# IRVLUTD/Proto-CLIP

Measured on AMD Instinct MI355X. Metric: query images/sec, ImageNet 16-shot ViT-B/16 (few-shot top-1 parity: tests/), higher is better.
Workload: dtype f16; 1 GPU; C3 ImageNet 16-shot ViT-B/16 conv-3x: prototype reduce + encode_image + adapter + dual-bank classify; batch_per_gpu=1024, global_batch=1024, classes=1000, shots=16, embed_dim=512, parallelism=dp1 (support rows and queries sharded; all-gather of class sums)

## Files before the change

### proto-clip_amd/csrc/pclip_attention.hip

```cpp
#include "pclip_attention_tile.h"
#include <stdlib.h>
#include <type_traits>

namespace {
constexpr int ATT_MAX_L = 288;

template <int NW, int VAR, bool QF = false>
__global__ __launch_bounds__(NW * 64, NW / 2) void attention_kernel(const half_t* __restrict__ qp, int ldq, long q_batch,
                                                           const half_t* __restrict__ kvp, int ldkv, int k_off, int v_off,
                                                           half_t* __restrict__ out, int L, int Lq, int H, int causal, int NT,
                                                           int LV) {
    extern __shared__ __attribute__((aligned(16))) char smem[];
    const int LP = NT * 32;
    half_t* Ks = reinterpret_cast<half_t*>(smem);
    half_t* Vs = Ks + LP * ATT_DH;
    const int b = blockIdx.x / H, h = blockIdx.x % H;
    const int W = H * ATT_DH;
    const half_t* kbase = kvp + (size_t)b * L * ldkv + h * ATT_DH + k_off;
    const half_t* vbase = kvp + (size_t)b * L * ldkv + h * ATT_DH + v_off;
    const half_t* qbase = qp + (size_t)b * q_batch + h * ATT_DH;
    const int tid = threadIdx.x, lane = tid & 63, wave = tid >> 6;
    half8_t qf0[4];
    if (QF) {
        const int q0 = wave * 32 + (lane & 31), qc0 = q0 < Lq ? q0 : Lq - 1;
#pragma unroll
        for (int s_ = 0; s_ < 4; ++s_) qf0[s_] = ld_half8(qbase + (size_t)qc0 * ldq + s_ * 16 + (lane >> 5) * 8);
    }

    for (int r0 = wave * 8; r0 < LP; r0 += NW * 8) {
        const int r = r0 + (lane >> 3);
        const int c = (lane & 7) ^ pgemm::swz_key(r);
        const int rc = r < L ? r : L - 1;
        __builtin_amdgcn_global_load_lds((pgemm::gbl_ptr_t)(kbase + (size_t)rc * ldkv + c * 8),
                                         (pgemm::lds_ptr_t)(Ks + r0 * ATT_DH), 16, 0, 0);
    }
    for (int r0 = wave * 8; r0 < LP; r0 += NW * 8) {
        const int r = r0 + (lane >> 3);
        const int c = (lane & 7) ^ (((r >> 1) & 1) << 2);
        const int rc = r < L ? r : L - 1;
        __builtin_amdgcn_global_load_lds((pgemm::gbl_ptr_t)(vbase + (size_t)rc * ldkv + c * 8),
                                         (pgemm::lds_ptr_t)(Vs + r0 * ATT_DH), 16, 0, 0);
    }
#ifndef PCLIP_ATT_VBAR
#define PCLIP_ATT_VBAR 1
#endif
    constexpr bool VB = PCLIP_ATT_VBAR && QF;
    if (VB) {
        const int nv = (LP - wave * 8 + NW * 8 - 1) / (NW * 8);
        if (nv <= 1) pgemm::wait_vm<1>(); else if (nv == 2) pgemm::wait_vm<2>(); else if (nv == 3) pgemm::wait_vm<3>(); else pgemm::wait_vm<4>();
        pgemm::lds_barrier();
    } else
        __syncthreads();

    const int hi = lane >> 5, ql = lane & 31;
    int voff[2];
    attn_voff(lane, voff);
    const int NTq = (Lq + 31) >> 5;
    auto process = [&](int qb, const half8_t (&qf)[4]) {
        const int q = qb * 32 + ql;
        float16_t o[2];
        float lrun;
        attn_query_tile<false, VAR, VB>(Ks, Vs, qf, q, qb, L, causal, NT, hi, ql, voff, o, lrun);
        attn_store_tile(out + ((size_t)b * Lq + q) * W + h * ATT_DH, o, lrun, hi, q < Lq);
    };
    if (QF) {
        if (wave < NTq) process(wave, qf0);
        else if (VB) { pgemm::wait_vm<0>(); pgemm::lds_barrier(); }
        return;
    }
    for (int qb = wave; qb < NTq; qb += NW) {
        const int q = qb * 32 + ql;
        const int qc = q < Lq ? q : Lq - 1;
        half8_t qf[4];
#pragma unroll
        for (int s = 0; s < 4; ++s) qf[s] = ld_half8(qbase + (size_t)qc * ldq + s * 16 + hi * 8);
        process(qb, qf);
    }
}

template <int NW, int WPS, int VAR>
__global__ __launch_bounds__(NW * 64, WPS) void attention_pipe_kernel(const half_t* __restrict__ qp, int ldq, long q_batch,
                                                                      const half_t* __restrict__ kvp, int ldkv, int k_off, int v_off,
                                                                      half_t* __restrict__ out, int L, int H, int causal, int NT, int KR,
                                                                      int nitems) {
    extern __shared__ __attribute__((aligned(16))) char smem[];
    constexpr int NST = 4;
    constexpr int MAXP = 4;
    constexpr int RB = ATT_DH * 2;
    const int LP = NT * 32;
    const int BUF = (KR + LP) * RB;
    const int tid = threadIdx.x, lane = tid & 63, wave = __builtin_amdgcn_readfirstlane(tid >> 6);
    const int hi = lane >> 5, ql = lane & 31;
    const int W = H * ATT_DH, G = gridDim.x;
    const bool has_tile = wave < NT;
    const unsigned lds0 = (unsigned)(size_t)(pgemm::lds_ptr_t)smem;
    char* Qs = smem + 2 * BUF;
    int voff[2];
    attn_voff(lane, voff);
    int kvo[MAXP], vvo[MAXP], qvo[MAXP];
#pragma unroll
    for (int i = 0; i < MAXP; ++i) {
        const int r = wave * 8 + i * NW * 8 + (lane >> 3);
        const int rc = r < L ? r : L - 1;
        const int ck = ((lane & 7) ^ pgemm::swz_key(r)) << 3, cv = ((lane & 7) ^ (((r >> 1) & 1) << 2)) << 3;
        kvo[i] = (rc * ldkv + ck) * 2;
        vvo[i] = (rc * ldkv + cv) * 2;
        qvo[i] = (rc * ldq + ck) * 2;
    }
    const int q = wave * 32 + ql;
    auto stage = [&](int item, int buf) {
        const int b = item / H, h = item - b * H;
        const uint4_t rkv = attn_rsrc(kvp + (size_t)b * L * ldkv + h * ATT_DH);
        const uint4_t rq = attn_rsrc(qp + (size_t)b * q_batch + h * ATT_DH);
        const unsigned kb = lds0 + buf * BUF, vb = kb + KR * RB, qb = lds0 + 2 * BUF;
#pragma unroll
        for (int i = 0; i < MAXP; ++i) {
            const int r0 = wave * 8 + i * NW * 8;
            if (r0 < KR) attn_dma16(rkv, kvo[i], k_off * 2, kb + r0 * RB);
        }
#pragma unroll
        for (int i = 0; i < MAXP; ++i) {
            const int r0 = wave * 8 + i * NW * 8;
            if (r0 < LP) attn_dma16(rkv, vvo[i], v_off * 2, vb + r0 * RB);
        }
#pragma unroll
        for (int i = 0; i < MAXP; ++i) {
            const int r0 = wave * 8 + i * NW * 8;
            if (r0 < KR) attn_dma16(rq, qvo[i], 0, qb + r0 * RB);
        }
    };
    int item = blockIdx.x;
    if (item >= nitems) return;
    stage(item, 0);
    for (int it = 0; item < nitems; item += G, ++it) {
        const int cur = it & 1;
        if (has_tile && it > 0) pgemm::wait_vm<NST>(); else pgemm::wait_vm<0>();
        pgemm::lds_barrier();
        half8_t qf[4];
        if (has_tile) {
            const int qr = q < KR ? q : KR - 1;
#pragma unroll
            for (int s = 0; s < 4; ++s)
                qf[s] = *reinterpret_cast<const half8_t*>(Qs + qr * RB + (((s * 2 + hi) ^ pgemm::swz_key(qr)) << 4));
        }
        pgemm::lds_barrier();
#ifndef PCLIP_ATT_ABL
#define PCLIP_ATT_ABL 0
#endif
        const int next = item + G;
        if (next < nitems && !(PCLIP_ATT_ABL & 1)) stage(next, cur ^ 1);
        if (has_tile) {
            const half_t* Ks = reinterpret_cast<const half_t*>(smem + cur * BUF);
            const half_t* Vs = Ks + KR * ATT_DH;
            float16_t o[2];
            float lrun;
#ifndef PCLIP_ATT_STAGGER
#define PCLIP_ATT_STAGGER 0
#endif
#if PCLIP_ATT_STAGGER && defined(__HIP_DEVICE_COMPILE__)
            if (wave >= NW / 2) __builtin_amdgcn_s_sleep(PCLIP_ATT_STAGGER);
#endif
            if (PCLIP_ATT_ABL & 2) {
#pragma unroll
                for (int j = 0; j < 2; ++j)
#pragma unroll
                    for (int e = 0; e < 16; ++e) o[j][e] = (float)qf[e & 3][e & 7];
                lrun = 1.f;
            } else
                attn_query_tile<true, VAR>(Ks, Vs, qf, q, wave, L, causal, NT, hi, ql, voff, o, lrun);
            const int b = item / H, h = item - b * H;
            attn_store_tile(out + ((size_t)b * L + q) * W + h * ATT_DH, o, lrun, hi, q < L && !(PCLIP_ATT_ABL & 4));
        }
    }
}

}

static int att_mode_from_env() {
    const char* e = getenv("PCLIP_ATT_PIPE");
    return e && (e[0] == '0' || e[0] == '1') ? e[0] - '0' : -1;
}
static int g_att_mode = att_mode_from_env(), g_att_grid = 0;
extern "C" int pclip_attention_config(int mode, int max_grid) {
    PCLIP_REQUIRE(mode >= -1 && mode <= 1 && max_grid >= 0, "pclip_attention_config: bad mode=%d max_grid=%d", mode, max_grid);
    g_att_mode = mode;
    g_att_grid = max_grid;
    return PCLIP_OK;
}

extern "C" int pclip_attention_q_f16(const void* q, int ldq, long q_batch_stride, const void* kv, int ldkv, int k_off, int v_off,
                                     void* out, int B, int L, int Lq, int H, int dh, int causal, pclip_stream_t stream) {
    PCLIP_REQUIRE(q && kv && out, "pclip_attention_q_f16: null pointer");
    PCLIP_REQUIRE(dh == ATT_DH, "pclip_attention_q_f16: head dim %d unsupported (must be 64)", dh);
    PCLIP_REQUIRE(B >= 0 && H > 0 && L > 0 && L <= ATT_MAX_L && Lq > 0 && Lq <= L, "pclip_attention_q_f16: bad B=%d H=%d L=%d Lq=%d (L <= %d)",
                  B, H, L, Lq, ATT_MAX_L);
    PCLIP_REQUIRE(!causal || Lq == L, "pclip_attention_q_f16: the causal mask needs all queries (Lq == L)");
    PCLIP_REQUIRE(ldq % 8 == 0 && ldkv % 8 == 0 && k_off % 8 == 0 && v_off % 8 == 0 && q_batch_stride % 8 == 0,
                  "pclip_attention_q_f16: strides / offsets must be multiples of 8 halves");
    if (B == 0) return PCLIP_OK;
    const int NT = ceil_div(L, 32), LP = NT * 32;
    const int LV = 0;
    const long nitems = (long)B * H;
    const int cus = pclip_device_cus();
    const int KR = (L + 7) / 8 * 8;
    const size_t plds = (2 * (size_t)(KR + LP) + KR) * ATT_DH * 2;
    if (Lq == L && g_att_mode != 0 && NT <= 8 && plds <= 160 * 1024 && cus > 0 && g_att_mode == 1) {
        static DevOnce pipe_attr;
        if (!pipe_attr.done()) {
            if (hipFuncSetAttribute((const void*)attention_pipe_kernel<4, 2, PCLIP_ATT_VAR_SHORT>, hipFuncAttributeMaxDynamicSharedMemorySize, 160 * 1024) != hipSuccess ||
                hipFuncSetAttribute((const void*)attention_pipe_kernel<8, 2, PCLIP_ATT_VAR_LONG>, hipFuncAttributeMaxDynamicSharedMemorySize, 160 * 1024) != hipSuccess) {
                pclip_set_error("pclip_attention_f16: cannot raise the dynamic LDS limit");
                return PCLIP_E_LAUNCH;
            }
            pipe_attr.set();
        }
        int per_cu = NT <= 4 ? (int)((160 * 1024) / plds) : 1;
        per_cu = per_cu < 1 ? 1 : (per_cu > 2 ? 2 : per_cu);
        long grid = (long)cus * per_cu;
        if (g_att_grid > 0 && g_att_grid < grid) grid = g_att_grid;
        if (grid > nitems) grid = nitems;
        if (NT <= 4)
            attention_pipe_kernel<4, 2, PCLIP_ATT_VAR_SHORT><<<(int)grid, 256, plds, (hipStream_t)stream>>>((const half_t*)q, ldq, q_batch_stride, (const half_t*)kv, ldkv,
                                                                                      k_off, v_off, (half_t*)out, L, H, causal, NT, KR, (int)nitems);
        else
            attention_pipe_kernel<8, 2, PCLIP_ATT_VAR_LONG><<<(int)grid, 512, plds, (hipStream_t)stream>>>((const half_t*)q, ldq, q_batch_stride, (const half_t*)kv, ldkv,
                                                                                      k_off, v_off, (half_t*)out, L, H, causal, NT, KR, (int)nitems);
        return pclip_check_launch("attention (pipelined)");
    }
    const size_t lds = 2 * (size_t)LP * ATT_DH * 2;
    static DevOnce attr_set;
    if (!attr_set.done()) {
        const void* fns[] = {(const void*)attention_kernel<8, PCLIP_ATT_VAR_LONG>, (const void*)attention_kernel<4, PCLIP_ATT_VAR_LONG>,
                             (const void*)attention_kernel<4, PCLIP_ATT_VAR_SHORT>, (const void*)attention_kernel<8, PCLIP_ATT_VAR_LONG, true>,
                             (const void*)attention_kernel<4, PCLIP_ATT_VAR_SHORT, true>};
        for (const void* f : fns)
            if (hipFuncSetAttribute(f, hipFuncAttributeMaxDynamicSharedMemorySize, 80 * 1024) != hipSuccess) {
                pclip_set_error("pclip_attention_f16: cannot raise the dynamic LDS limit");
                return PCLIP_E_LAUNCH;
            }
        attr_set.set();
    }
#define PCLIP_ATT_LAUNCH(NW, VAR)                                                                                                         \
    attention_kernel<NW, VAR><<<B * H, NW * 64, lds, (hipStream_t)stream>>>((const half_t*)q, ldq, q_batch_stride, (const half_t*)kv, ldkv, k_off, \
                                                                             v_off, (half_t*)out, L, Lq, H, causal, NT, LV)
    static const bool qfirst = !(getenv("PCLIP_ATT_QFIRST") && getenv("PCLIP_ATT_QFIRST")[0] == '0');
    if (PCLIP_ATT_QF4 && qfirst && NT <= 4 && Lq == L && !causal)
        attention_kernel<4, PCLIP_ATT_VAR_SHORT, true><<<B * H, 4 * 64, lds, (hipStream_t)stream>>>((const half_t*)q, ldq, q_batch_stride, (const half_t*)kv, ldkv, k_off,
                                                                                                     v_off, (half_t*)out, L, Lq, H, causal, NT, LV);
    else if ((Lq + 31) / 32 > 4 && (Lq + 31) / 32 <= 8 && NT <= 8 && qfirst)
        attention_kernel<8, PCLIP_ATT_VAR_LONG, true><<<B * H, 8 * 64, lds, (hipStream_t)stream>>>((const half_t*)q, ldq, q_batch_stride, (const half_t*)kv, ldkv, k_off,
                                                                                                    v_off, (half_t*)out, L, Lq, H, causal, NT, LV);
    else if ((Lq + 31) / 32 > 4) PCLIP_ATT_LAUNCH(8, PCLIP_ATT_VAR_LONG);
    else if (NT > 4) PCLIP_ATT_LAUNCH(4, PCLIP_ATT_VAR_LONG);
    else PCLIP_ATT_LAUNCH(4, PCLIP_ATT_VAR_SHORT);
#undef PCLIP_ATT_LAUNCH
    return pclip_check_launch("attention");
}

extern "C" int pclip_attention_f16(const void* qkv, void* out, int B, int L, int H, int dh, int causal,
                                   pclip_stream_t stream) {
    PCLIP_REQUIRE(qkv && out, "pclip_attention_f16: null pointer");
    PCLIP_REQUIRE(H > 0 && L > 0, "pclip_attention_f16: bad H=%d L=%d", H, L);
    const int W = H * dh;
    return pclip_attention_q_f16(qkv, 3 * W, (long)L * 3 * W, qkv, 3 * W, W, 2 * W, out, B, L, L, H, dh, causal, stream);
}
```

### proto-clip_amd/csrc/pclip_attention_tile.h

```cpp
#pragma once
#include "pclip_encoder_common.h"
#include <type_traits>

namespace {
constexpr int ATT_DH = 64;
constexpr float kAttDefer = 2.f;
#ifndef PCLIP_ATT_VAR_LONG
#define PCLIP_ATT_VAR_LONG 15
#endif
#ifndef PCLIP_ATT_VAR_SHORT
#define PCLIP_ATT_VAR_SHORT 1
#endif

typedef __fp16 fp16x4_t __attribute__((__vector_size__(4 * sizeof(__fp16))));
__device__ __forceinline__ half4_t tr_read4(const char* lds_addr) {
    const fp16x4_t v = __builtin_amdgcn_ds_read_tr16_b64_v4f16((__attribute__((address_space(3))) fp16x4_t*)(lds_addr));
    return __builtin_bit_cast(half4_t, v);
}

__device__ __forceinline__ void attn_voff(int lane, int (&voff)[2]) {
    const int hi = lane >> 5;
    const int i16 = lane & 15, vrow = hi * 4 + (i16 >> 2), vd = ((lane >> 4) & 1) * 16 + 4 * (i16 & 3), vswz = ((vrow >> 1) & 1) << 2;
#pragma unroll
    for (int j = 0; j < 2; ++j) voff[j] = vrow * (ATT_DH * 2) + ((((j * 4 + (vd >> 3)) ^ vswz)) << 4) + (vd & 7) * 2;
}

__device__ __forceinline__ void half_wave_pair(float v, float& r0, float& r1) {
#if defined(__HIP_DEVICE_COMPILE__)
    const unsigned a = __builtin_bit_cast(unsigned, v);
    const auto r = __builtin_amdgcn_permlane32_swap(a, a, false, false);
    const unsigned x = r[0], y = r[1];
    r0 = __builtin_bit_cast(float, x);
    r1 = __builtin_bit_cast(float, y);
#else
    r0 = r1 = v;
#endif
}
__device__ __forceinline__ float half_wave_max(float v) { float a, b; half_wave_pair(v, a, b); return fmaxf(a, b); }
__device__ __forceinline__ float half_wave_sum(float v) { float a, b; half_wave_pair(v, a, b); return a + b; }

#ifndef PCLIP_ATT_QF4
#define PCLIP_ATT_QF4 1
#endif
#ifndef PCLIP_ATT_EDGE
#define PCLIP_ATT_EDGE 1
#endif
template <bool DEEP = false, int VAR = 0, bool VBAR = false>
__device__ __forceinline__ void attn_key_tiles(const half_t* Ks, const half_t* Vs, const half8_t (&qf)[4], int q, int qb, int L, int causal,
                                               int NT, int hi, int ql, const int (&voff)[2], float16_t (&o)[2],
                                               float& mrun_io, float& lrun_io) {
    constexpr float kScale = 0.125f * 1.4426950408889634f;
    float mrun = mrun_io, lrun = lrun_io;
    const int tend = causal ? (qb + 1 < NT ? qb + 1 : NT) : NT;
    auto k_frag = [&](int t, int sidx) {
        const int kr = t * 32 + ql;
        return *reinterpret_cast<const half8_t*>(Ks + kr * ATT_DH + (((sidx * 2 + hi) ^ pgemm::swz_key(kr)) << 3));
    };
    auto v_frag = [&](int t, int sidx, int j) {
        const char* vb = reinterpret_cast<const char*>(Vs) + (t * 32 + sidx * 16) * (ATT_DH * 2) + voff[j];
        const half4_t v0 = tr_read4(vb);
        const half4_t v1 = tr_read4(vb + 8 * (ATT_DH * 2));
        return half8_t{v0[0], v0[1], v0[2], v0[3], v1[0], v1[1], v1[2], v1[3]};
    };
    half8_t kpre[2][4];
    auto k_prefetch = [&](int t0) {
#pragma unroll
        for (int u = 0; u < 2; ++u) {
            const int tt = t0 + u < NT ? t0 + u : NT - 1;
#pragma unroll
            for (int sidx = 0; sidx < 4; ++sidx) kpre[u][sidx] = k_frag(tt, sidx);
        }
    };
    auto tiles = [&](auto NTILE_C, int t0) {
        constexpr int NTILE = decltype(NTILE_C)::value;
        float16_t st[NTILE];
#pragma unroll
        for (int u = 0; u < NTILE; ++u)
#pragma unroll
            for (int e = 0; e < 16; ++e) st[u][e] = 0.f;
#if defined(__HIP_DEVICE_COMPILE__)
        if (VAR & 8) __builtin_amdgcn_s_setprio(1);
#endif
#pragma unroll
        for (int sidx = 0; sidx < 4; ++sidx)
#pragma unroll
            for (int u = 0; u < NTILE; ++u) {
                const half8_t kf = DEEP ? kpre[u][sidx] : k_frag(t0 + u, sidx);
                st[u] = __builtin_amdgcn_mfma_f32_32x32x16_f16(kf, qf[sidx], st[u], 0, 0, 0);
            }
#if defined(__HIP_DEVICE_COMPILE__)
        if (VAR & 8) __builtin_amdgcn_s_setprio(0);
#endif
        half8_t vpre[NTILE][2][2];
        if (DEEP) {
#pragma unroll
            for (int u = 0; u < NTILE; ++u)
#pragma unroll
                for (int sidx = 0; sidx < 2; ++sidx)
#pragma unroll
                    for (int j = 0; j < 2; ++j) vpre[u][sidx][j] = v_frag(t0 + u, sidx, j);
            const int tn = t0 + NTILE;
            if (tn < tend) k_prefetch(tn);
#if defined(__HIP_DEVICE_COMPILE__)
            __builtin_amdgcn_sched_barrier(0);
#endif
        }
        float tmax = -__builtin_inff();
#pragma unroll
        for (int u = 0; u < NTILE; ++u) {
            const int t = t0 + u;
            if ((t * 32 + 32 > L) || (causal && t == qb)) {
                const int kend = causal ? (q + 1 < L ? q + 1 : L) : L;
                const int lim = kend - t * 32 - 4 * hi;
#pragma unroll
                for (int e = 0; e < 16; ++e)
                    if (!((e & 3) + 8 * (e >> 2) < lim)) st[u][e] = -__builtin_inff();
            }
        }
        {
            float m4[4] = {tmax, tmax, tmax, tmax};
#pragma unroll
            for (int u = 0; u < NTILE; ++u)
#pragma unroll
                for (int e = 0; e < 16; ++e) m4[e & 3] = fmaxf(m4[e & 3], st[u][e]);
            tmax = fmaxf(fmaxf(m4[0], m4[1]), fmaxf(m4[2], m4[3]));
        }
        tmax = half_wave_max(tmax) * kScale;
        const bool moved = (VAR & 1) ? tmax > mrun + kAttDefer : fmaxf(mrun, tmax) != mrun;
        const float mnew = ((VAR & 1) && !moved) ? mrun : fmaxf(mrun, tmax);
        const bool grow = __any(moved);
        float psum = 0.f;
        if (VAR & 6) {
            float2_t ps2 = {0.f, 0.f};
            const float2_t ks2 = {kScale, kScale}, nm2 = {-mnew, -mnew};
#pragma unroll
            for (int u = 0; u < NTILE; ++u)
#pragma unroll
                for (int e = 0; e < 16; e += 2) {
                    float2_t v = {st[u][e], st[u][e + 1]};
                    if (VAR & 4) {
                        v = v * ks2 + nm2;
                        v = float2_t{__builtin_amdgcn_exp2f(v[0]), __builtin_amdgcn_exp2f(v[1])};
                    } else
                        v = float2_t{__builtin_amdgcn_exp2f(fmaf(v[0], kScale, -mnew)), __builtin_amdgcn_exp2f(fmaf(v[1], kScale, -mnew))};
                    st[u][e] = v[0];
                    st[u][e + 1] = v[1];
                    if (VAR & 2) ps2 += v;
                    else { psum += v[0]; psum += v[1]; }
                }
            psum += ps2[0] + ps2[1];
        } else {
#pragma unroll
            for (int u = 0; u < NTILE; ++u)
#pragma unroll
                for (int e = 0; e < 16; ++e) { st[u][e] = __builtin_amdgcn_exp2f(fmaf(st[u][e], kScale, -mnew)); psum += st[u][e]; }
        }
        psum = half_wave_sum(psum);
        if (grow) {
            const float alpha = __builtin_amdgcn_exp2f(mrun - mnew);
            lrun *= alpha;
#pragma unroll
            for (int j = 0; j < 2; ++j)
#pragma unroll
                for (int e = 0; e < 16; ++e) o[j][e] *= alpha;
        }
        lrun += psum;
        mrun = mnew;
        if (VBAR && t0 == 0) { pgemm::wait_vm<0>(); pgemm::lds_barrier(); }
#pragma unroll
        for (int u = 0; u < NTILE; ++u)
#pragma unroll
            for (int sidx = 0; sidx < 2; ++sidx) {
                half8_t pf;
#pragma unroll
                for (int e = 0; e < 8; ++e) pf[e] = (half_t)st[u][sidx * 8 + e];
#if defined(__HIP_DEVICE_COMPILE__)
                if (VAR & 8) __builtin_amdgcn_s_setprio(1);
#endif
#pragma unroll
                for (int j = 0; j < 2; ++j) {
                    const half8_t vf = DEEP ? vpre[u][sidx][j] : v_frag(t0 + u, sidx, j);
                    o[j] = __builtin_amdgcn_mfma_f32_32x32x16_f16(vf, pf, o[j], 0, 0, 0);
                }
#if defined(__HIP_DEVICE_COMPILE__)
                if (VAR & 8) __builtin_amdgcn_s_setprio(0);
#endif
            }
    };
    auto tile_edge = [&](int t0) {
        const int ng = (L - t0 * 32 + 7) >> 3;
        float16_t st;
#pragma unroll
        for (int e = 0; e < 16; ++e) st[e] = 0.f;
#if defined(__HIP_DEVICE_COMPILE__)
        if (VAR & 8) __builtin_amdgcn_s_setprio(1);
#endif
#pragma unroll
        for (int sidx = 0; sidx < 4; ++sidx) st = __builtin_amdgcn_mfma_f32_32x32x16_f16(k_frag(t0, sidx), qf[sidx], st, 0, 0, 0);
#if defined(__HIP_DEVICE_COMPILE__)
        if (VAR & 8) __builtin_amdgcn_s_setprio(0);
#endif
        const int lim = L - t0 * 32 - 4 * hi;
        float m4[4] = {-__builtin_inff(), -__builtin_inff(), -__builtin_inff(), -__builtin_inff()};
#pragma unroll
        for (int g = 0; g < 3; ++g)
            if (g < ng) {
#pragma unroll
                for (int r = 0; r < 4; ++r) {
                    if (!(r + 8 * g < lim)) st[4 * g + r] = -__builtin_inff();
                    m4[r] = fmaxf(m4[r], st[4 * g + r]);
                }
            }
        float tmax = fmaxf(fmaxf(m4[0], m4[1]), fmaxf(m4[2], m4[3]));
        tmax = half_wave_max(tmax) * kScale;
        const bool moved = (VAR & 1) ? tmax > mrun + kAttDefer : fmaxf(mrun, tmax) != mrun;
        const float mnew = ((VAR & 1) && !moved) ? mrun : fmaxf(mrun, tmax);
        const bool grow = __any(moved);
        float psum = 0.f;
        float2_t ps2 = {0.f, 0.f};
        const float2_t ks2 = {kScale, kScale}, nm2 = {-mnew, -mnew};
#pragma unroll
        for (int g = 0; g < 4; ++g) {
            if (g < 3 && g < ng) {
#pragma unroll
                for (int e = 4 * g; e < 4 * g + 4; e += 2) {
                    float2_t v = {st[e], st[e + 1]};
                    if (VAR & 6) {
                        if (VAR & 4) {
                            v = v * ks2 + nm2;
                            v = float2_t{__builtin_amdgcn_exp2f(v[0]), __builtin_amdgcn_exp2f(v[1])};
                        } else
                            v = float2_t{__builtin_amdgcn_exp2f(fmaf(v[0], kScale, -mnew)), __builtin_amdgcn_exp2f(fmaf(v[1], kScale, -mnew))};
                        if (VAR & 2) ps2 += v;
                        else { psum += v[0]; psum += v[1]; }
                    } else {
                        v[0] = __builtin_amdgcn_exp2f(fmaf(v[0], kScale, -mnew)); psum += v[0];
                        v[1] = __builtin_amdgcn_exp2f(fmaf(v[1], kScale, -mnew)); psum += v[1];
                    }
                    st[e] = v[0];
                    st[e + 1] = v[1];
                }
            } else {
#pragma unroll
                for (int r = 0; r < 4; ++r) st[4 * g + r] = 0.f;
            }
        }
        if (VAR & 6) psum += ps2[0] + ps2[1];
        psum = half_wave_sum(psum);
        if (grow) {
            const float alpha = __builtin_amdgcn_exp2f(mrun - mnew);
            lrun *= alpha;
#pragma unroll
            for (int j = 0; j < 2; ++j)
#pragma unroll
                for (int e = 0; e < 16; ++e) o[j][e] *= alpha;
        }
        lrun += psum;
        mrun = mnew;
        if (VBAR && t0 == 0) { pgemm::wait_vm<0>(); pgemm::lds_barrier(); }
#pragma unroll
        for (int sidx = 0; sidx < 2; ++sidx)
            if (sidx == 0 || ng > 2) {
                half8_t pf;
#pragma unroll
                for (int e = 0; e < 8; ++e) pf[e] = (half_t)st[sidx * 8 + e];
#if defined(__HIP_DEVICE_COMPILE__)
                if (VAR & 8) __builtin_amdgcn_s_setprio(1);
#endif
#pragma unroll
                for (int j = 0; j < 2; ++j) o[j] = __builtin_amdgcn_mfma_f32_32x32x16_f16(v_frag(t0, sidx, j), pf, o[j], 0, 0, 0);
#if defined(__HIP_DEVICE_COMPILE__)
                if (VAR & 8) __builtin_amdgcn_s_setprio(0);
#endif
            }
    };
    int t = 0;
    if (DEEP) k_prefetch(0);
    for (; t + 1 < tend; t += 2) tiles(std::integral_constant<int, 2>{}, t);
    if (t < tend) {
        if (PCLIP_ATT_EDGE && VBAR && !DEEP && !causal && L - t * 32 <= 24) tile_edge(t);
        else tiles(std::integral_constant<int, 1>{}, t);
    }
    mrun_io = mrun;
    lrun_io = lrun;
}

template <bool DEEP = false, int VAR = 0, bool VBAR = false>
__device__ __forceinline__ void attn_query_tile(const half_t* Ks, const half_t* Vs, const half8_t (&qf)[4], int q, int qb, int L, int causal,
                                                int NT, int hi, int ql, const int (&voff)[2], float16_t (&o)[2], float& lrun_out) {
#pragma unroll
    for (int j = 0; j < 2; ++j)
#pragma unroll
        for (int e = 0; e < 16; ++e) o[j][e] = 0.f;
    float mrun = -__builtin_inff(), lrun = 0.f;
    attn_key_tiles<DEEP, VAR, VBAR>(Ks, Vs, qf, q, qb, L, causal, NT, hi, ql, voff, o, mrun, lrun);
    lrun_out = lrun;
}

__device__ __forceinline__ void attn_store_tile(half_t* orow, const float16_t (&o)[2], float lrun, int hi, bool valid) {
    const float inv = 1.f / lrun;
#pragma unroll
    for (int j = 0; j < 2; ++j)
#pragma unroll
        for (int k = 0; k < 2; ++k) {
            unsigned a[2], bq[2];
#pragma unroll
            for (int w = 0; w < 2; ++w) {
                const half2_t ha = {(half_t)(o[j][8 * k + 2 * w] * inv), (half_t)(o[j][8 * k + 2 * w + 1] * inv)};
                const half2_t hb = {(half_t)(o[j][8 * k + 4 + 2 * w] * inv), (half_t)(o[j][8 * k + 4 + 2 * w + 1] * inv)};
                a[w] = __builtin_bit_cast(unsigned, ha);
                bq[w] = __builtin_bit_cast(unsigned, hb);
            }
#if defined(__HIP_DEVICE_COMPILE__)
#pragma unroll
            for (int w = 0; w < 2; ++w) {
                const auto r = __builtin_amdgcn_permlane32_swap(a[w], bq[w], false, false);
                a[w] = r[0];
                bq[w] = r[1];
            }
#endif
            if (valid) *reinterpret_cast<uint4_t*>(orow + j * 32 + 16 * k + 8 * hi) = uint4_t{a[0], a[1], bq[0], bq[1]};
        }
}

__device__ __forceinline__ void attn_dma16(uint4_t rs, int voff, int soff, unsigned lds_addr) {
#if defined(__HIP_DEVICE_COMPILE__)
    unsigned keep;
    asm volatile(
        "s_nop 4\n\t"
        "s_mov_b32 %0, m0\n\t"
        "s_mov_b32 m0, %3\n\t"
        "s_nop 0\n\t"
        "buffer_load_dwordx4 %1, %2, %4 offen lds\n\t"
        "s_mov_b32 m0, %0"
        : "=&s"(keep)
        : "v"(voff), "s"(rs), "s"(lds_addr), "s"(soff)
        : "memory");
#endif
}
__device__ __forceinline__ uint4_t attn_rsrc(const void* base) {
    const uint64_t addr = (uint64_t)base;
    const uint32_t lo = __builtin_amdgcn_readfirstlane((uint32_t)addr), hi = __builtin_amdgcn_readfirstlane((uint32_t)(addr >> 32));
    return uint4_t{lo, hi & 0xffffu, 0x7fffffffu, 0x00020000u};
}

}
```

Measured before the change: 28980 query images/sec.

## Stream K/V tiles into LDS via direct DMA with per-pair arrival waits in attention

Adds an attention kernel variant that issues every K/V row load up front as buffer-to-LDS DMA and loads Q into registers with raw buffer loads. Each pair of key tiles then waits only on its own outstanding loads before computing, so QK/PV math on early tiles overlaps the arrival of later tiles instead of waiting on a full-tile barrier. This path is used for non-causal sequences longer than 128 keys, which covers ViT-B/16's 197 tokens. In exchange it relies on hand-counted vmcnt waits and inline asm, and the 4-wave case now uses the LONG variant.

```diff
diff --git a/proto-clip_amd/csrc/pclip_attention.hip b/proto-clip_amd/csrc/pclip_attention.hip
--- a/proto-clip_amd/csrc/pclip_attention.hip
+++ b/proto-clip_amd/csrc/pclip_attention.hip
@@ -5,12 +5,80 @@
 namespace {
 constexpr int ATT_MAX_L = 288;
 
-template <int NW, int VAR, bool QF = false>
+template <int NW>
+struct AttnPairArrival {
+    static constexpr bool kArrival = true;
+    int nv;
+    __device__ __forceinline__ void wait(int p) const {
+        const int upto = (p + 1) * (8 / NW) < nv ? (p + 1) * (8 / NW) : nv;
+        attn_wait_vm_even<NW == 8 ? 6 : 14>(2 * (nv - upto));
+    }
+    __device__ __forceinline__ void operator()(int p) const {
+        if (p > 0) { wait(p); pgemm::lds_barrier(); }
+    }
+};
+template <int NW, int VAR>
+__device__ __forceinline__ void attention_arrival(const half_t* __restrict__ qp, int ldq, long q_batch, const half_t* __restrict__ kvp, int ldkv, int k_off, int v_off,
+                                                  half_t* __restrict__ out, int L, int Lq, int H, int NT, char* smem) {
+    constexpr int PP = 8 / NW;
+    constexpr int MAXPAIR = NW == 8 ? 4 : 5;
+    constexpr int RB = ATT_DH * 2;
+    const int LP = NT * 32;
+    const int b = blockIdx.x / H, h = blockIdx.x % H;
+    const int W = H * ATT_DH;
+    const int tid = threadIdx.x, lane = tid & 63, wave = __builtin_amdgcn_readfirstlane(tid >> 6);
+    const int hi = lane >> 5, ql = lane & 31;
+    const int q = wave * 32 + ql, qc = q < Lq ? q : Lq - 1;
+    uint4_t qr[4];
+    attn_load_q(attn_rsrc(qp + (size_t)b * q_batch + h * ATT_DH), (qc * ldq + hi * 8) * 2, qr);
+    const uint4_t rkv = attn_rsrc(kvp + (size_t)b * L * ldkv + h * ATT_DH);
+    const unsigned ks = (unsigned)(size_t)(pgemm::lds_ptr_t)smem, vs = ks + LP * RB;
+#pragma unroll
+    for (int p = 0; p < MAXPAIR; ++p) {
+#pragma unroll
+        for (int op = 0; op < 2; ++op)
+#pragma unroll
+            for (int j = 0; j < PP; ++j) {
+                const int r0 = wave * 8 + NW * 8 * (p * PP + j);
+                if (r0 < LP) {
+                    const int r = r0 + (lane >> 3);
+                    const int rc = r < L ? r : L - 1;
+                    const int c = (lane & 7) ^ (op == 0 ? pgemm::swz_key(r) : ((r >> 1) & 1) << 2);
+                    attn_dma16(rkv, (rc * ldkv + c * 8) * 2, (op == 0 ? k_off : v_off) * 2, (op == 0 ? ks : vs) + r0 * RB);
+                }
+            }
+    }
+    const AttnPairArrival<NW> arrive{(LP - wave * 8 + NW * 8 - 1) / (NW * 8)};
+    arrive.wait(0);
+    attn_pin_q(qr);
+    pgemm::lds_barrier();
+    const int NP = (NT + 1) >> 1;
+    if (wave < ((Lq + 31) >> 5)) {
+        const half_t* Ks = reinterpret_cast<const half_t*>(smem);
+        const half_t* Vs = Ks + LP * ATT_DH;
+        half8_t qf[4];
+#pragma unroll
+        for (int s_ = 0; s_ < 4; ++s_) qf[s_] = __builtin_bit_cast(half8_t, qr[s_]);
+        int voff[2];
+        attn_voff(lane, voff);
+        float16_t o[2];
+        float lrun;
+        attn_query_tile<false, VAR, false>(Ks, Vs, qf, q, wave, L, 0, NT, hi, ql, voff, o, lrun, arrive);
+        attn_store_tile(out + ((size_t)b * Lq + q) * W + h * ATT_DH, o, lrun, hi, q < Lq);
+    } else
+        for (int p = 1; p < NP; ++p) arrive(p);
+}
+
+template <int NW, int VAR, bool QF = false, bool ARR = false>
 __global__ __launch_bounds__(NW * 64, NW / 2) void attention_kernel(const half_t* __restrict__ qp, int ldq, long q_batch,
                                                            const half_t* __restrict__ kvp, int ldkv, int k_off, int v_off,
                                                            half_t* __restrict__ out, int L, int Lq, int H, int causal, int NT,
                                                            int LV) {
     extern __shared__ __attribute__((aligned(16))) char smem[];
+    if (ARR) {
+        attention_arrival<NW, VAR>(qp, ldq, q_batch, kvp, ldkv, k_off, v_off, out, L, Lq, H, NT, smem);
+        return;
+    }
     const int LP = NT * 32;
     half_t* Ks = reinterpret_cast<half_t*>(smem);
     half_t* Vs = Ks + LP * ATT_DH;
@@ -232,7 +300,8 @@
     if (!attr_set.done()) {
         const void* fns[] = {(const void*)attention_kernel<8, PCLIP_ATT_VAR_LONG>, (const void*)attention_kernel<4, PCLIP_ATT_VAR_LONG>,
                              (const void*)attention_kernel<4, PCLIP_ATT_VAR_SHORT>, (const void*)attention_kernel<8, PCLIP_ATT_VAR_LONG, true>,
-                             (const void*)attention_kernel<4, PCLIP_ATT_VAR_SHORT, true>};
+                             (const void*)attention_kernel<4, PCLIP_ATT_VAR_SHORT, true>, (const void*)attention_kernel<8, PCLIP_ATT_VAR_LONG, true, true>,
+                             (const void*)attention_kernel<4, PCLIP_ATT_VAR_LONG, true, true>};
         for (const void* f : fns)
             if (hipFuncSetAttribute(f, hipFuncAttributeMaxDynamicSharedMemorySize, 80 * 1024) != hipSuccess) {
                 pclip_set_error("pclip_attention_f16: cannot raise the dynamic LDS limit");
@@ -244,7 +313,15 @@
     attention_kernel<NW, VAR><<<B * H, NW * 64, lds, (hipStream_t)stream>>>((const half_t*)q, ldq, q_batch_stride, (const half_t*)kv, ldkv, k_off, \
                                                                              v_off, (half_t*)out, L, Lq, H, causal, NT, LV)
     static const bool qfirst = !(getenv("PCLIP_ATT_QFIRST") && getenv("PCLIP_ATT_QFIRST")[0] == '0');
-    if (PCLIP_ATT_QF4 && qfirst && NT <= 4 && Lq == L && !causal)
+    const int NTq = (Lq + 31) / 32;
+    const bool arr = qfirst && !causal && NT > 4 && (long)L * ldkv * 2 < 0x7fffffffL && (long)Lq * ldq * 2 < 0x7fffffffL;
+    if (arr && NTq > 4 && NTq <= 8 && NT <= 8)
+        attention_kernel<8, PCLIP_ATT_VAR_LONG, true, true><<<B * H, 8 * 64, lds, (hipStream_t)stream>>>((const half_t*)q, ldq, q_batch_stride, (const half_t*)kv, ldkv, k_off,
+                                                                                                          v_off, (half_t*)out, L, Lq, H, causal, NT, LV);
+    else if (arr && NTq <= 4)
+        attention_kernel<4, PCLIP_ATT_VAR_LONG, true, true><<<B * H, 4 * 64, lds, (hipStream_t)stream>>>((const half_t*)q, ldq, q_batch_stride, (const half_t*)kv, ldkv, k_off,
+                                                                                                          v_off, (half_t*)out, L, Lq, H, causal, NT, LV);
+    else if (PCLIP_ATT_QF4 && qfirst && NT <= 4 && Lq == L && !causal)
         attention_kernel<4, PCLIP_ATT_VAR_SHORT, true><<<B * H, 4 * 64, lds, (hipStream_t)stream>>>((const half_t*)q, ldq, q_batch_stride, (const half_t*)kv, ldkv, k_off,
                                                                                                      v_off, (half_t*)out, L, Lq, H, causal, NT, LV);
     else if ((Lq + 31) / 32 > 4 && (Lq + 31) / 32 <= 8 && NT <= 8 && qfirst)
diff --git a/proto-clip_amd/csrc/pclip_attention_tile.h b/proto-clip_amd/csrc/pclip_attention_tile.h
--- a/proto-clip_amd/csrc/pclip_attention_tile.h
+++ b/proto-clip_amd/csrc/pclip_attention_tile.h
@@ -45,10 +45,14 @@
 #ifndef PCLIP_ATT_EDGE
 #define PCLIP_ATT_EDGE 1
 #endif
-template <bool DEEP = false, int VAR = 0, bool VBAR = false>
+struct AttnNoArrival {
+    static constexpr bool kArrival = false;
+    __device__ __forceinline__ void operator()(int) const {}
+};
+template <bool DEEP = false, int VAR = 0, bool VBAR = false, class ARRIVE = AttnNoArrival>
 __device__ __forceinline__ void attn_key_tiles(const half_t* Ks, const half_t* Vs, const half8_t (&qf)[4], int q, int qb, int L, int causal,
                                                int NT, int hi, int ql, const int (&voff)[2], float16_t (&o)[2],
-                                               float& mrun_io, float& lrun_io) {
+                                               float& mrun_io, float& lrun_io, ARRIVE arrive = ARRIVE{}) {
     constexpr float kScale = 0.125f * 1.4426950408889634f;
     float mrun = mrun_io, lrun = lrun_io;
     const int tend = causal ? (qb + 1 < NT ? qb + 1 : NT) : NT;
@@ -78,6 +82,7 @@
         for (int u = 0; u < NTILE; ++u)
 #pragma unroll
             for (int e = 0; e < 16; ++e) st[u][e] = 0.f;
+        arrive(t0 >> 1);
 #if defined(__HIP_DEVICE_COMPILE__)
         if (VAR & 8) __builtin_amdgcn_s_setprio(1);
 #endif
@@ -192,6 +197,7 @@
         float16_t st;
 #pragma unroll
         for (int e = 0; e < 16; ++e) st[e] = 0.f;
+        arrive(t0 >> 1);
 #if defined(__HIP_DEVICE_COMPILE__)
         if (VAR & 8) __builtin_amdgcn_s_setprio(1);
 #endif
@@ -278,22 +284,22 @@
     if (DEEP) k_prefetch(0);
     for (; t + 1 < tend; t += 2) tiles(std::integral_constant<int, 2>{}, t);
     if (t < tend) {
-        if (PCLIP_ATT_EDGE && VBAR && !DEEP && !causal && L - t * 32 <= 24) tile_edge(t);
+        if (PCLIP_ATT_EDGE && (VBAR || ARRIVE::kArrival) && !DEEP && !causal && L - t * 32 <= 24) tile_edge(t);
         else tiles(std::integral_constant<int, 1>{}, t);
     }
     mrun_io = mrun;
     lrun_io = lrun;
 }
 
-template <bool DEEP = false, int VAR = 0, bool VBAR = false>
+template <bool DEEP = false, int VAR = 0, bool VBAR = false, class ARRIVE = AttnNoArrival>
 __device__ __forceinline__ void attn_query_tile(const half_t* Ks, const half_t* Vs, const half8_t (&qf)[4], int q, int qb, int L, int causal,
-                                                int NT, int hi, int ql, const int (&voff)[2], float16_t (&o)[2], float& lrun_out) {
+                                                int NT, int hi, int ql, const int (&voff)[2], float16_t (&o)[2], float& lrun_out, ARRIVE arrive = ARRIVE{}) {
 #pragma unroll
     for (int j = 0; j < 2; ++j)
 #pragma unroll
         for (int e = 0; e < 16; ++e) o[j][e] = 0.f;
     float mrun = -__builtin_inff(), lrun = 0.f;
-    attn_key_tiles<DEEP, VAR, VBAR>(Ks, Vs, qf, q, qb, L, causal, NT, hi, ql, voff, o, mrun, lrun);
+    attn_key_tiles<DEEP, VAR, VBAR>(Ks, Vs, qf, q, qb, L, causal, NT, hi, ql, voff, o, mrun, lrun, arrive);
     lrun_out = lrun;
 }
 
@@ -343,5 +349,35 @@
     const uint32_t lo = __builtin_amdgcn_readfirstlane((uint32_t)addr), hi = __builtin_amdgcn_readfirstlane((uint32_t)(addr >> 32));
     return uint4_t{lo, hi & 0xffffu, 0x7fffffffu, 0x00020000u};
 }
-
-}
+__device__ __forceinline__ void attn_load_q(uint4_t rs, int voff, uint4_t (&qr)[4]) {
+#if defined(__HIP_DEVICE_COMPILE__)
+    asm volatile(
+        "s_nop 4\n\t"
+        "buffer_load_dwordx4 %0, %4, %5, 0 offen\n\t"
+        "buffer_load_dwordx4 %1, %4, %5, 0 offen offset:32\n\t"
+        "buffer_load_dwordx4 %2, %4, %5, 0 offen offset:64\n\t"
+        "buffer_load_dwordx4 %3, %4, %5, 0 offen offset:96"
+        : "=&v"(qr[0]), "=&v"(qr[1]), "=&v"(qr[2]), "=&v"(qr[3])
+        : "v"(voff), "s"(rs)
+        : "memory");
+#endif
+}
+__device__ __forceinline__ void attn_pin_q(uint4_t (&qr)[4]) {
+#if defined(__HIP_DEVICE_COMPILE__)
+    asm volatile("" : "+v"(qr[0]), "+v"(qr[1]), "+v"(qr[2]), "+v"(qr[3]) : : "memory");
+#endif
+}
+template <int MAXN>
+__device__ __forceinline__ void attn_wait_vm_even(int n) {
+    static_assert(MAXN <= 14, "add the cases");
+    if (MAXN >= 14 && n == 14) pgemm::wait_vm<14>();
+    else if (MAXN >= 12 && n == 12) pgemm::wait_vm<12>();
+    else if (MAXN >= 10 && n == 10) pgemm::wait_vm<10>();
+    else if (MAXN >= 8 && n == 8) pgemm::wait_vm<8>();
+    else if (MAXN >= 6 && n == 6) pgemm::wait_vm<6>();
+    else if (MAXN >= 4 && n == 4) pgemm::wait_vm<4>();
+    else if (MAXN >= 2 && n == 2) pgemm::wait_vm<2>();
+    else pgemm::wait_vm<0>();
+}
+
+}
```

Measured after the change: 29040 query images/sec (median of 6 runs). About the same (+0.2%).
